# foldl/chatllm.cpp

Measured on AMD Instinct MI355X. Metric: decode tokens/s, higher is better.
Workload: dtype int8xint4 dot / f32 accumulate (Q8_K x Q4_K); 1 GPU; llama3-8b shapes, Q4_K weights, single-token decode, batch 1, 16-token prompt, F16 KV cache; parallelism=single GPU, n_ctx_end=1630

## Files before the change

chatllm.cpp_amd/csrc/decode_fused.hip:

```cpp
#include "common.h"
#include "quant_dev.h"
#include "q4k.h"
#include "dequant.h"

#include <math.h>

__device__ __forceinline__ float lane_xor4_ff(float v) { return __int_as_float(lane_xor4_i(__float_as_int(v))); }
__device__ __forceinline__ float vd32_reduce(float a0, float a1) {
    a0 = a0 + dpp_f<DPP_ROW_ROR8>(a0); a1 = a1 + dpp_f<DPP_ROW_ROR8>(a1);
    a0 = a0 + lane_xor4_ff(a0);        a1 = a1 + lane_xor4_ff(a1);
    a0 = a0 + dpp_f<DPP_QUAD_XOR2>(a0); a1 = a1 + dpp_f<DPP_QUAD_XOR2>(a1);
    const float u = a0 + a1;
    return u + dpp_f<DPP_QUAD_XOR1>(u);
}

static float * g_attn_dbg = nullptr;
static unsigned long long * g_attn_ts = nullptr;
extern "C" __attribute__((visibility("default"))) void cllm_debug_set_attn_ts(unsigned long long * dev_buf) { g_attn_ts = dev_buf; }
extern "C" __attribute__((visibility("default"))) void cllm_debug_set_attn_probs(float * dev_buf) { g_attn_dbg = dev_buf; }

template <bool ROPE>
__global__ void __launch_bounds__(1024) k_attn_decode(const float * __restrict__ qkv, const int32_t * __restrict__ pos_dev, int nh, int nkv, int hd,
                                                      float scale, uint16_t * __restrict__ k_cache, uint16_t * __restrict__ v_cache,
                                                      int64_t ML, float * __restrict__ att, float * __restrict__ dbg, int mode, float theta_scale) {
// ... 118 lines not shown
    const int np = n_kv & ~31, ntail = n_kv - np;
    for (int d0 = wave * 4 + sub; d0 < hd; d0 += nrg) {
        const uint16_t * vr = v_cache + ((int64_t) g * hd + d0) * ML;
        const float vfresh = ROPE ? vnew[d0] : 0.0f;
        float a0 = 0.0f, a1 = 0.0f;
        for (int e = 2 * c16; e < np; e += 32) {
            const float v0 = (ROPE && e == pos) ? vfresh : h2f(vr[e]), v1 = (ROPE && e + 1 == pos) ? vfresh : h2f(vr[e + 1]);
            a0 = __builtin_fmaf(v0, sc[e], a0); a1 = __builtin_fmaf(v1, sc[e + 1], a1);
        }
        const float res = vd32_reduce(a0, a1);
        for (int t = 0; t < 2; t++) {
            const int e = np + 2 * c16 + t;
            if (e < n_kv) tailp[2 * c16 + t] = ((ROPE && e == pos) ? vfresh : h2f(vr[e])) * sc[e];
        }
        wave_lds_fence();
        if (c16 == 0) {
            double s = (double) res;
            for (int t = 0; t < ntail; t++) s += (double) tailp[t];
            att[h * hd + d0] = (float) s;
        }
        wave_lds_fence();
    }
}

__global__ void __launch_bounds__(64) k_rope_table(const int32_t * __restrict__ pos_dev, int half, float theta_scale, float * __restrict__ cs) {
    for (int i = threadIdx.x; i < half; i += 64) {
        float theta = (float) pos_dev[0];
        for (int k = 0; k < i; k++) theta *= theta_scale;
        float c, s_;
        rope_cos_sin(theta, &c, &s_);
        cs[2*i] = c * 1.0f; cs[2*i + 1] = s_ * 1.0f;
    }
}
int launch_rope_table(hipStream_t st, const int32_t * pos_dev, int hd, float freq_base, float * cs) {
    hipLaunchKernelGGL(k_rope_table, dim3(1), dim3(64), 0, st, pos_dev, hd / 2, powf(freq_base, -2.0f / hd), cs);
    LAUNCH_CHECK();
    return CLLM_OK;
}

__device__ __forceinline__ int uniform_load_i32(const int32_t * p) {
    int v;
    asm volatile("s_load_dword %0, %1, 0x0\n\ts_waitcnt lgkmcnt(0)" : "=s"(v) : "s"(p) : "memory");
    return v;
}

template <int HD, int MODE, int PARTS>
__global__ void __launch_bounds__(1024) k_attn_dec(const float * __restrict__ qkv, const int32_t * __restrict__ pos_dev, const float * __restrict__ rope_cs,
                                                   int nh, int nkv, float scale, uint16_t * __restrict__ k_cache, uint16_t * __restrict__ v_cache,
                                                   int ML, float * __restrict__ att, unsigned long long * ts) {
#define TS(k) do { if (ts && threadIdx.x == 0) ts[(blockIdx.y * gridDim.x + blockIdx.x) * 8 + (k)] = wall_clock64(); } while (0)
    extern __shared__ __attribute__((aligned(16))) float sm[];
    __shared__ float  red_f[16];
    __shared__ uint64_t etab_s[32];
    constexpr int half = HD / 2, off = MODE == 0 ? 1 : half, U = 4;
    const int r2 = gridDim.x, g = blockIdx.y, h = g * r2 + blockIdx.x;
    const int tid = threadIdx.x, lane = tid & 63, wave = tid >> 6;
    const int KD = nkv * HD, QD = nh * HD;
    float * qs = sm; float * knew = sm + HD; float * vnew = sm + 2 * HD; float * sc = sm + 3 * HD;

    float px0 = 0.0f, px1 = 0.0f, pc = 0.0f, ps = 0.0f;
    const bool is_pair = tid < 2 * half, is_v = !is_pair && tid < 2 * half + HD;
    const int which = tid >= half ? 1 : 0, pi = tid - which * half, ic = MODE == 0 ? 2 * pi : pi;
    if (is_pair) {
        const float * x = which == 0 ? qkv + h * HD : qkv + QD + g * HD;
        px0 = x[ic]; px1 = x[ic + off];
        pc = rope_cs[2 * pi]; ps = rope_cs[2 * pi + 1];
    } else if (is_v) px0 = qkv[QD + KD + g * HD + (tid - 2 * half)];
    const int pos = uniform_load_i32(pos_dev);
// ... 251 lines not shown
__global__ void __launch_bounds__(256) k_argmax_partial(const float * __restrict__ x, int n, float * __restrict__ pv, int * __restrict__ pi) {
    __shared__ float bv[4]; __shared__ int bi[4];
    const int per = (n + gridDim.x - 1) / gridDim.x;
    const int lo = blockIdx.x * per, hi = min(n, lo + per);
    float best = -INFINITY; int idx = 0x7fffffff;
    for (int i = lo + threadIdx.x; i < hi; i += 256) { const float v = x[i]; if (v > best) { best = v; idx = i; } }
#pragma unroll
    for (int o = 32; o > 0; o >>= 1) argmax_combine(best, idx, __shfl_xor(best, o, 64), __shfl_xor(idx, o, 64));
    if ((threadIdx.x & 63) == 0) { bv[threadIdx.x >> 6] = best; bi[threadIdx.x >> 6] = idx; }
    __syncthreads();
    if (threadIdx.x == 0) {
        for (int w = 1; w < 4; w++) argmax_combine(best, idx, bv[w], bi[w]);
        pv[blockIdx.x] = best; pi[blockIdx.x] = idx;
    }
}
__global__ void __launch_bounds__(256) k_argmax_final(const float * __restrict__ pv, const int * __restrict__ pi, int np, int32_t * __restrict__ tok_dev,
                                                      int32_t * __restrict__ pos_dev, int32_t * __restrict__ out_ring, int32_t * __restrict__ counter) {
    __shared__ float bv[4]; __shared__ int bi[4];
    float best = -INFINITY; int idx = 0x7fffffff;
    for (int i = threadIdx.x; i < np; i += 256) argmax_combine(best, idx, pv[i], pi[i]);
#pragma unroll
    for (int o = 32; o > 0; o >>= 1) argmax_combine(best, idx, __shfl_xor(best, o, 64), __shfl_xor(idx, o, 64));
    if ((threadIdx.x & 63) == 0) { bv[threadIdx.x >> 6] = best; bi[threadIdx.x >> 6] = idx; }
    __syncthreads();
    if (threadIdx.x == 0) {
        for (int w = 1; w < 4; w++) argmax_combine(best, idx, bv[w], bi[w]);
        if (idx == 0x7fffffff) idx = 0;
        tok_dev[0] = idx;
        pos_dev[0] = pos_dev[0] + 1;
        out_ring[counter[0]] = idx;
        counter[0] = counter[0] + 1;
    }
}
__global__ void __launch_bounds__(1024) k_argmax_final_next(const float * __restrict__ pv, const int * __restrict__ pi, int np, int32_t * __restrict__ tok_dev,
                                                            int32_t * __restrict__ pos_dev, int32_t * __restrict__ out_ring, int32_t * __restrict__ counter,
                                                            int etype, const char * __restrict__ emb, size_t emb_nb1, int H, float * __restrict__ x_next,
                                                            int half, float theta_scale, float * __restrict__ cs) {
    __shared__ float bv[16]; __shared__ int bi[16]; __shared__ int tok_s;
    const int tid = threadIdx.x;
    const int pos_next = pos_dev[0] + 1;
    float best = -INFINITY; int idx = 0x7fffffff;
    for (int i = tid; i < np; i += 1024) argmax_combine(best, idx, pv[i], pi[i]);
#pragma unroll
    for (int o = 32; o > 0; o >>= 1) argmax_combine(best, idx, __shfl_xor(best, o, 64), __shfl_xor(idx, o, 64));
    if ((tid & 63) == 0) { bv[tid >> 6] = best; bi[tid >> 6] = idx; }
    __syncthreads();
    if (tid == 0) {
        for (int w = 1; w < 16; w++) argmax_combine(best, idx, bv[w], bi[w]);
        if (idx == 0x7fffffff) idx = 0;
        tok_s = idx;
        tok_dev[0] = idx;
        pos_dev[0] = pos_next;
        out_ring[counter[0]] = idx;
        counter[0] = counter[0] + 1;
    }
    if (cs && tid >= 960)
        for (int i = tid - 960; i < half; i += 64) {
            float theta = (float) pos_next;
            for (int k = 0; k < i; k++) theta *= theta_scale;
            float c, s_;
            rope_cos_sin(theta, &c, &s_);
            cs[2*i] = c * 1.0f; cs[2*i + 1] = s_ * 1.0f;
        }
    __syncthreads();
    const char * row = emb + (size_t) tok_s * emb_nb1;
    for (int c = tid; c < H; c += 1024) x_next[c] = dequant_elem(etype, row, c);
}
int launch_argmax_partial(hipStream_t st, const float * logits, int n, float * part_v, int * part_i) {
    hipLaunchKernelGGL(k_argmax_partial, dim3(256), dim3(256), 0, st, logits, n, part_v, part_i);
    LAUNCH_CHECK();
    return CLLM_OK;
}
int launch_argmax_final_next(hipStream_t st, const float * part_v, const int * part_i, int np, int32_t * tok_dev, int32_t * pos_dev, int32_t * out_ring, int32_t * counter,
                             int etype, const void * emb, size_t emb_nb1, int H, float * x_next, int hd, float freq_base, float * cs) {
    hipLaunchKernelGGL(k_argmax_final_next, dim3(1), dim3(1024), 0, st, part_v, part_i, np, tok_dev, pos_dev, out_ring, counter, etype, (const char *) emb, emb_nb1, H, x_next,
                       hd / 2, hd ? powf(freq_base, -2.0f / hd) : 0.0f, hd ? cs : (float *) nullptr);
    LAUNCH_CHECK();
    return CLLM_OK;
}
__global__ void __launch_bounds__(256) k_argmax_publish(const float * __restrict__ pv, const int * __restrict__ pi, int np, int32_t * __restrict__ tok_dev,
                                                        int32_t * __restrict__ tok_host, int32_t * const * __restrict__ inc, int n_inc) {
    __shared__ float bv[4]; __shared__ int bi[4];
    float best = -INFINITY; int idx = 0x7fffffff;
    for (int i = threadIdx.x; i < np; i += 256) argmax_combine(best, idx, pv[i], pi[i]);
#pragma unroll
    for (int o = 32; o > 0; o >>= 1) argmax_combine(best, idx, __shfl_xor(best, o, 64), __shfl_xor(idx, o, 64));
    if ((threadIdx.x & 63) == 0) { bv[threadIdx.x >> 6] = best; bi[threadIdx.x >> 6] = idx; }
    __syncthreads();
    if (threadIdx.x == 0) {
        for (int w = 1; w < 4; w++) argmax_combine(best, idx, bv[w], bi[w]);
        if (idx == 0x7fffffff) idx = 0;
        tok_dev[0] = idx;
        if (tok_host) { tok_host[0] = idx; __threadfence_system(); }
    }
    for (int i = threadIdx.x; i < n_inc; i += 256) inc[i][0] = inc[i][0] + 1;
}
struct argmax_set_rec { int32_t * ptr; int32_t val; int32_t pad; };
__global__ void __launch_bounds__(256) k_argmax_publish_set(const float * __restrict__ pv, const int * __restrict__ pi, int np, int32_t * __restrict__ tok_dev,
                                                            int32_t * __restrict__ tok_host, const argmax_set_rec * __restrict__ recs, int n_set) {
    __shared__ float bv[4]; __shared__ int bi[4];
    float best = -INFINITY; int idx = 0x7fffffff;
    for (int i = threadIdx.x; i < np; i += 256) argmax_combine(best, idx, pv[i], pi[i]);
#pragma unroll
    for (int o = 32; o > 0; o >>= 1) argmax_combine(best, idx, __shfl_xor(best, o, 64), __shfl_xor(idx, o, 64));
    if ((threadIdx.x & 63) == 0) { bv[threadIdx.x >> 6] = best; bi[threadIdx.x >> 6] = idx; }
    __syncthreads();
    if (threadIdx.x == 0) {
        for (int w = 1; w < 4; w++) argmax_combine(best, idx, bv[w], bi[w]);
        if (idx == 0x7fffffff) idx = 0;
        tok_dev[0] = idx;
        if (tok_host) { tok_host[0] = idx; __threadfence_system(); }
// ... 88 lines not shown
```

chatllm.cpp_amd/lib.py:

```python
import ctypes as C
import os
import subprocess

HERE = os.path.dirname(os.path.abspath(__file__))
SO_PATH = os.environ.get("CLLM_LIB") or os.path.join(HERE, "libchatllm_hip.so")
HEADER = os.path.join(os.path.dirname(HERE), "include", "chatllm_hip.h")


class CllmError(RuntimeError):

    def __init__(self, msg, rc=None):
        super().__init__(msg)
        self.rc = rc


class CTensor(C.Structure):
    _fields_ = [("type", C.c_int32), ("ne", C.c_int64 * 4), ("nb", C.c_size_t * 4), ("data", C.c_void_p)]


class RopeParams(C.Structure):
    _fields_ = [("n_dims", C.c_int32), ("mode", C.c_int32), ("n_ctx_orig", C.c_int32), ("freq_base", C.c_float),
                ("freq_scale", C.c_float), ("ext_factor", C.c_float), ("attn_factor", C.c_float),
                ("beta_fast", C.c_float), ("beta_slow", C.c_float)]

# ... 36 lines not shown
    "cllm_scratch_release": (C.c_int, [_P]),
    "cllm_check_kernel_errors": (C.c_int, []),
    "cllm_graph_capture_begin": (C.c_int, [_P]),
    "cllm_graph_capture_end": (C.c_int, [_P, C.POINTER(C.c_void_p)]),
    "cllm_graph_launch": (C.c_int, [_P, _P]),
    "cllm_graph_destroy": (C.c_int, [_P]),
    "cllm_event_create": (C.c_int, [C.POINTER(C.c_void_p)]),
    "cllm_event_destroy": (C.c_int, [_P]),
    "cllm_event_record": (C.c_int, [_P, _P]),
    "cllm_event_sync": (C.c_int, [_P]),
    "cllm_stream_wait_event": (C.c_int, [_P, _P]),
    "cllm_memcpy_peer_async": (C.c_int, [_P, C.c_int, _P, C.c_int, C.c_size_t, _P]),
    "cllm_event_elapsed_ms": (C.c_int, [_P, _P, C.POINTER(C.c_float)]),
    "cllm_mul_mat_wsize": (C.c_size_t, [_T, _T]),
    "cllm_op_mul_mat": (C.c_int, [_P, _T, _T, _T, _P, C.c_size_t]),
    "cllm_mul_mat_ex_min_cols": (C.c_int, []),
    "cllm_set_prefill_mode": (C.c_int, [C.c_int]),
    "cllm_get_prefill_mode": (C.c_int, []),
    "cllm_set_prefill_attn_mode": (C.c_int, [C.c_int]),
    "cllm_op_mul_mat_ex": (C.c_int, [_P, _T, _T, _T, _P, C.c_size_t, C.c_int, _T, C.c_float, C.c_int, _T]),
    "cllm_set_decode_free_order": (C.c_int, [C.c_int]),
    "cllm_get_decode_free_order": (C.c_int, []),
    "cllm_op_mul_mat_vec_fused": (C.c_int, [_P, _T, C.c_int, _P, _P, C.c_float, C.c_int, _P, _P]),
    "cllm_pack_rows": (C.c_int, [_P, _P, C.POINTER(C.c_void_p), C.POINTER(C.c_int64), C.c_int, C.c_size_t, C.c_int]),
    "cllm_bench_mul_mat_kernel": (C.c_int, [_P, _T, C.POINTER(C.c_void_p), C.c_int, _T, _T, _P, C.c_size_t, C.c_int, C.POINTER(C.c_float)]),
    "cllm_bench_mul_mat_id": (C.c_int, [_P, _T, _T, _T, C.POINTER(C.c_void_p), C.c_int, _T, _P, C.c_size_t, C.c_int, C.POINTER(C.c_float)]),
    "cllm_bench_read_bw": (C.c_int, [_P, C.c_size_t, C.c_int, C.POINTER(C.c_float)]),
    "cllm_bench_gemv_fused": (C.c_int, [_P, C.c_int, C.POINTER(C.c_void_p), C.c_int, C.c_int64, C.c_int64, C.c_int, _P, _P, C.c_float, C.c_int, _P, _P, C.c_int,
                                        C.POINTER(C.c_float)]),
    "cllm_op_mul_mat_id": (C.c_int, [_P, _T, _T, _T, _T, _P, C.c_size_t]),
    "cllm_op_argmax_advance": (C.c_int, [_P, _P, C.c_int64, _P, _P, _P, C.c_int, _P]),
    "cllm_op_argmax_set": (C.c_int, [_P, _P, C.c_int64, _P, _P, _P, C.c_int, _P]),
    "cllm_op_snapshot_argmax_set": (C.c_int, [_P, _P, C.c_int, _P, C.c_int64, _P, _P, _P, C.c_int, _P]),
    "cllm_flash_attn_wsize": (C.c_size_t, [_T]),
    "cllm_op_flash_attn_ext": (C.c_int, [_P, _T, _T, _T, _T, _T, C.c_float, C.c_float, C.c_float, _P, C.c_size_t]),
    "cllm_attn_prefill_min_cols": (C.c_int, []),
    "cllm_op_attn_prefill": (C.c_int, [_P, _T, _T, _T, _T, C.c_float, C.c_int]),
    "cllm_op_mul_mat_id_silu_mul": (C.c_int, [_P, _T, _T, _T, _T]),
    "cllm_quantize_row_q8_0": (C.c_int, [_P, _P, _P, C.c_int64]),
    "cllm_quantize_row_q8_1": (C.c_int, [_P, _P, _P, C.c_int64]),
    "cllm_quantize_row_q8_K": (C.c_int, [_P, _P, _P, C.c_int64]),
    "cllm_vec_dot_isums": (C.c_int, [_P, C.c_int, C.c_int64, _P, _P, _P]),
    "cllm_op_rms_norm": (C.c_int, [_P, _T, _T, C.c_float]),
    "cllm_op_rms_norm_mul": (C.c_int, [_P, _T, _T, _T, C.c_float]),
    "cllm_op_rope": (C.c_int, [_P, _T, _T, _T, _T, C.POINTER(RopeParams)]),
    "cllm_op_soft_max": (C.c_int, [_P, _T, _T, _T, C.c_float, C.c_float]),
    "cllm_op_diag_mask_inf": (C.c_int, [_P, _T, _T, C.c_int]),
    "cllm_op_scale": (C.c_int, [_P, _T, _T, C.c_float, C.c_float]),
    "cllm_op_scale_mask_soft_max": (C.c_int, [_P, _T, _T, C.c_float, C.c_int]),
    "cllm_op_attn_decode": (C.c_int, [_P, _P, _P, C.c_int, C.c_int, C.c_int, _P, _P, C.c_int64, _P]),
    "cllm_op_rope_table": (C.c_int, [_P, _P, C.c_int, C.c_float, _P]),
    "cllm_attn_decode_supported": (C.c_int, [C.c_int, C.c_int, C.c_int, C.c_int64]),
    "cllm_attn_decode_wsize": (C.c_size_t, [C.c_int64, C.c_int, C.c_int64]),
    "cllm_op_rope_kv_attn_decode": (C.c_int, [_P, _P, _P, _P, C.c_float, C.c_int64, C.c_int, C.c_int, C.c_int, C.c_int, _P, _P, C.c_int64, _P, _P, C.c_size_t]),
    "cllm_op_unary": (C.c_int, [_P, C.c_int, _T, _T]),
    "cllm_op_sqr": (C.c_int, [_P, _T, _T]),
    "cllm_op_add": (C.c_int, [_P, _T, _T, _T]),
    "cllm_op_mul": (C.c_int, [_P, _T, _T, _T]),
    "cllm_op_div": (C.c_int, [_P, _T, _T, _T]),
    "cllm_op_sum_rows": (C.c_int, [_P, _T, _T]),
    "cllm_op_top_k": (C.c_int, [_P, _T, _T]),
    "cllm_op_moe_combine": (C.c_int, [_P, _T, _T, _T, _T, _T]),
    "cllm_op_mul_mat_id_combine": (C.c_int, [_P, _T, _T, _T, _T, _T, _T]),
    "cllm_op_moe_router": (C.c_int, [_P, _T, _T, C.c_float, _T, _T, _T, _T]),
    "cllm_op_moe_router_gate_up": (C.c_int, [_P, _T, _T, C.c_float, _T, _T, _T, _T, _T]),
    "cllm_op_silu_mul": (C.c_int, [_P, _T, _T, _T]),
# ... 92 lines not shown
```

include/chatllm_hip.h:

```cpp
#ifndef CHATLLM_HIP_H
#define CHATLLM_HIP_H

#include <stddef.h>
#include <stdint.h>

#ifdef __cplusplus
extern "C" {
#endif

#define CLLM_API __attribute__((visibility("default")))

typedef enum cllm_status {
    CLLM_OK            =  0,
    CLLM_E_INVALID     = -1,
    CLLM_E_UNSUPPORTED = -2,
    CLLM_E_HIP         = -3,
    CLLM_E_ALLOC       = -4,
} cllm_status;

typedef enum cllm_type {
    CLLM_TYPE_F32 = 0, CLLM_TYPE_F16 = 1, CLLM_TYPE_Q4_0 = 2, CLLM_TYPE_Q4_1 = 3, CLLM_TYPE_Q8_0 = 8, CLLM_TYPE_Q4_K = 12, CLLM_TYPE_Q5_K = 13, CLLM_TYPE_Q6_K = 14,
    CLLM_TYPE_Q5_0 = 6, CLLM_TYPE_Q5_1 = 7, CLLM_TYPE_Q2_K = 10, CLLM_TYPE_Q3_K = 11, CLLM_TYPE_IQ4_NL = 20, CLLM_TYPE_IQ2_XXS = 16, CLLM_TYPE_IQ2_XS = 17, CLLM_TYPE_IQ3_XXS = 18, CLLM_TYPE_IQ1_S = 19, CLLM_TYPE_IQ3_S = 21, CLLM_TYPE_IQ2_S = 22, CLLM_TYPE_IQ4_XS = 23, CLLM_TYPE_IQ1_M = 29, CLLM_TYPE_TQ1_0 = 34, CLLM_TYPE_TQ2_0 = 35, CLLM_TYPE_MXFP4 = 39,
    CLLM_TYPE_I32 = 26, CLLM_TYPE_I64 = 27,
} cllm_type;
// ... 80 lines not shown

CLLM_API int    cllm_quantize_row_q8_0(void * stream, const float * x, void * y_blocks, int64_t k);
CLLM_API int    cllm_quantize_row_q8_1(void * stream, const float * x, void * y_blocks, int64_t k);
CLLM_API int    cllm_quantize_row_q8_K(void * stream, const float * x, void * y_blocks, int64_t k);
CLLM_API int    cllm_vec_dot_isums(void * stream, int wtype, int64_t k, const void * w_row, const float * x, int32_t * isums);

CLLM_API int cllm_op_rms_norm(void * stream, const cllm_tensor * src, cllm_tensor * dst, float eps);
CLLM_API int cllm_op_rms_norm_mul(void * stream, const cllm_tensor * src, const cllm_tensor * weight, cllm_tensor * dst, float eps);

typedef struct cllm_rope_params {
    int32_t n_dims, mode, n_ctx_orig;
    float   freq_base, freq_scale, ext_factor, attn_factor, beta_fast, beta_slow;
} cllm_rope_params;
CLLM_API int cllm_op_rope(void * stream, const cllm_tensor * src, const cllm_tensor * pos, const cllm_tensor * freq_factors,
                          cllm_tensor * dst, const cllm_rope_params * p);
CLLM_API int cllm_op_soft_max(void * stream, const cllm_tensor * src, const cllm_tensor * mask, cllm_tensor * dst,
                              float scale, float max_bias);
CLLM_API int cllm_op_diag_mask_inf(void * stream, const cllm_tensor * src, cllm_tensor * dst, int n_past);
CLLM_API int cllm_op_scale(void * stream, const cllm_tensor * src, cllm_tensor * dst, float s, float b);
CLLM_API int cllm_op_scale_mask_soft_max(void * stream, const cllm_tensor * src, cllm_tensor * dst, float scale, int n_past);

CLLM_API size_t cllm_flash_attn_wsize(const cllm_tensor * q);
CLLM_API int    cllm_op_flash_attn_ext(void * stream, const cllm_tensor * q, const cllm_tensor * k, const cllm_tensor * v, const cllm_tensor * mask,
                                       cllm_tensor * dst, float scale, float max_bias, float logit_softcap, void * wdata, size_t wsize);
CLLM_API int    cllm_attn_prefill_min_cols(void);
CLLM_API int    cllm_op_attn_prefill(void * stream, const cllm_tensor * q, const cllm_tensor * k, const cllm_tensor * vt, cllm_tensor * dst,
                                     float scale, int n_past);

CLLM_API int cllm_op_argmax_advance(void * stream, const float * logits, int64_t n, int32_t * tok_dev, int32_t * tok_host,
                                    int32_t * const * inc_ptrs_dev, int n_inc, void * scratch);
CLLM_API int cllm_op_argmax_set(void * stream, const float * logits, int64_t n, int32_t * tok_dev, int32_t * tok_host, const void * set_table_dev, int n_set, void * scratch);
CLLM_API int cllm_op_snapshot_argmax_set(void * stream, const void * ranges_dev, int n_ranges, const float * logits, int64_t n, int32_t * tok_dev, int32_t * tok_host,
                                         const void * set_table_dev, int n_set, void * scratch);

CLLM_API int cllm_op_attn_decode(void * stream, const float * q, const int32_t * pos_dev, int n_head, int n_kv_head, int head_dim,
                                 const void * k_cache, const void * v_cache, int64_t max_len, float * out);

CLLM_API int    cllm_op_rope_table(void * stream, const int32_t * pos_dev, int head_dim, float freq_base, float * cs );
CLLM_API int    cllm_attn_decode_supported(int n_head, int n_kv_head, int head_dim, int64_t max_len);
CLLM_API size_t cllm_attn_decode_wsize(int64_t n_kv, int n_head, int64_t max_len);
CLLM_API int    cllm_op_rope_kv_attn_decode(void * stream, const float * qkv, const int32_t * pos_dev, const float * rope_cs, float freq_base, int64_t n_kv,
                                            int n_head, int n_kv_head, int head_dim, int rope_mode, void * k_cache, void * v_cache, int64_t max_len,
                                            float * out, void * wdata, size_t wsize);

typedef enum cllm_unary {
    CLLM_UNARY_TANH = 4, CLLM_UNARY_RELU = 6, CLLM_UNARY_SIGMOID = 7, CLLM_UNARY_GELU = 8, CLLM_UNARY_GELU_QUICK = 9, CLLM_UNARY_SILU = 10,
} cllm_unary;
CLLM_API int cllm_op_unary(void * stream, int op, const cllm_tensor * src, cllm_tensor * dst);
CLLM_API int cllm_op_sqr(void * stream, const cllm_tensor * src, cllm_tensor * dst);
CLLM_API int cllm_op_add(void * stream, const cllm_tensor * a, const cllm_tensor * b, cllm_tensor * dst);
CLLM_API int cllm_op_mul(void * stream, const cllm_tensor * a, const cllm_tensor * b, cllm_tensor * dst);
CLLM_API int cllm_op_div(void * stream, const cllm_tensor * a, const cllm_tensor * b, cllm_tensor * dst);
CLLM_API int cllm_op_sum_rows(void * stream, const cllm_tensor * src, cllm_tensor * dst);
CLLM_API int cllm_op_top_k(void * stream, const cllm_tensor * src, cllm_tensor * dst);
CLLM_API int cllm_op_moe_combine(void * stream, const cllm_tensor * experts, const cllm_tensor * probs, const cllm_tensor * ids, const cllm_tensor * resid,
                                 cllm_tensor * dst);
CLLM_API int cllm_op_mul_mat_id_combine(void * stream, const cllm_tensor * as, const cllm_tensor * b, const cllm_tensor * ids, const cllm_tensor * probs,
                                        const cllm_tensor * resid, cllm_tensor * dst);
CLLM_API int cllm_op_moe_router_gate_up(void * stream, const cllm_tensor * x, const cllm_tensor * norm_w, float eps, const cllm_tensor * gate_w, const cllm_tensor * as_gu,
                                        cllm_tensor * probs, cllm_tensor * ids, cllm_tensor * dst);
CLLM_API int cllm_op_moe_router(void * stream, const cllm_tensor * x, const cllm_tensor * norm_w, float eps, const cllm_tensor * gate_w,
                                cllm_tensor * xnorm, cllm_tensor * probs, cllm_tensor * ids);
CLLM_API int cllm_op_silu_mul(void * stream, const cllm_tensor * gate, const cllm_tensor * up, cllm_tensor * dst);

CLLM_API int cllm_op_set_rows(void * stream, const cllm_tensor * src, const cllm_tensor * idx, cllm_tensor * dst);
CLLM_API int cllm_op_cpy(void * stream, const cllm_tensor * src, cllm_tensor * dst);
// ... 68 lines not shown
```

Baseline: 667.3 tokens/s.

## Specialize argmax-final-next kernel per embedding type with warp-split roles and LDS row staging

Adds a templated 320-thread version of the final argmax kernel. Four wavefronts reduce the argmax in a single shuffle pass and stage the chosen embedding row in LDS, while a fifth wavefront advances the position and computes the rope table concurrently. Q4_K rows are dequantized eight values per thread with vectorized stores, which replaces the per-element dequant over 1024 threads and one of the barriers. The change also adds timestamp probes, a flag to force the generic path, and public C entry points; the kernel is one small launch per token, so its effect on overall decode speed is limited.

```diff
diff --git a/chatllm.cpp_amd/csrc/decode_fused.hip b/chatllm.cpp_amd/csrc/decode_fused.hip
--- a/chatllm.cpp_amd/csrc/decode_fused.hip
+++ b/chatllm.cpp_amd/csrc/decode_fused.hip
@@ -493,19 +493,29 @@
         counter[0] = counter[0] + 1;
     }
 }
+static unsigned long long * g_final_ts = nullptr;
+static bool g_final_generic = false;
+extern "C" __attribute__((visibility("default"))) void cllm_debug_set_final_ts(unsigned long long * dev_buf) { g_final_ts = dev_buf; }
+extern "C" __attribute__((visibility("default"))) void cllm_debug_set_final_generic(int on) { g_final_generic = on != 0; }
+#define FTS(k) do { if (ts) ts[(k)] = wall_clock64(); } while (0)
 __global__ void __launch_bounds__(1024) k_argmax_final_next(const float * __restrict__ pv, const int * __restrict__ pi, int np, int32_t * __restrict__ tok_dev,
                                                             int32_t * __restrict__ pos_dev, int32_t * __restrict__ out_ring, int32_t * __restrict__ counter,
                                                             int etype, const char * __restrict__ emb, size_t emb_nb1, int H, float * __restrict__ x_next,
-                                                            int half, float theta_scale, float * __restrict__ cs) {
+                                                            int half, float theta_scale, float * __restrict__ cs, unsigned long long * __restrict__ ts) {
     __shared__ float bv[16]; __shared__ int bi[16]; __shared__ int tok_s;
     const int tid = threadIdx.x;
+    unsigned long long * const ts_all = ts;
+    if (tid) ts = nullptr;
+    FTS(0);
     const int pos_next = pos_dev[0] + 1;
     float best = -INFINITY; int idx = 0x7fffffff;
     for (int i = tid; i < np; i += 1024) argmax_combine(best, idx, pv[i], pi[i]);
 #pragma unroll
     for (int o = 32; o > 0; o >>= 1) argmax_combine(best, idx, __shfl_xor(best, o, 64), __shfl_xor(idx, o, 64));
     if ((tid & 63) == 0) { bv[tid >> 6] = best; bi[tid >> 6] = idx; }
-    __syncthreads();
+    FTS(1);
+    __syncthreads();
+    FTS(2);
     if (tid == 0) {
         for (int w = 1; w < 16; w++) argmax_combine(best, idx, bv[w], bi[w]);
         if (idx == 0x7fffffff) idx = 0;
@@ -515,7 +525,8 @@
         out_ring[counter[0]] = idx;
         counter[0] = counter[0] + 1;
     }
-    if (cs && tid >= 960)
+    FTS(3);
+    if (cs && tid >= 960) {
         for (int i = tid - 960; i < half; i += 64) {
             float theta = (float) pos_next;
             for (int k = 0; k < i; k++) theta *= theta_scale;
@@ -523,19 +534,136 @@
             rope_cos_sin(theta, &c, &s_);
             cs[2*i] = c * 1.0f; cs[2*i + 1] = s_ * 1.0f;
         }
-    __syncthreads();
+        if (ts_all && tid == 960) ts_all[6] = wall_clock64();
+    }
+    __syncthreads();
+    FTS(4);
     const char * row = emb + (size_t) tok_s * emb_nb1;
     for (int c = tid; c < H; c += 1024) x_next[c] = dequant_elem(etype, row, c);
+    FTS(5);
 }
 int launch_argmax_partial(hipStream_t st, const float * logits, int n, float * part_v, int * part_i) {
     hipLaunchKernelGGL(k_argmax_partial, dim3(256), dim3(256), 0, st, logits, n, part_v, part_i);
     LAUNCH_CHECK();
     return CLLM_OK;
 }
+static __device__ __noinline__ float2 rope_cos_sin_v(float theta) {
+    float2 r;
+    r.x = gm_cosf(theta);
+    r.y = gm_sinf(theta);
+    return r;
+}
+__device__ __forceinline__ void q4k_row_decode8(const char * row, int g, float * __restrict__ x) {
+    const uint32_t * blk = (const uint32_t *)(row + (size_t)(g >> 5) * 144);
+    const int r = g & 31, j = r >> 3, l = (r & 7) * 4;
+    const uint32_t dm = blk[0], s0 = blk[1], s1 = blk[2], s2 = blk[3], q = blk[4 + 8 * j + (r & 7)];
+    auto sb = [&](int i) { const uint32_t w = i < 4 ? s0 : i < 8 ? s1 : s2; return (int)((w >> (8 * (i & 3))) & 0xff); };
+    float d1[2], m1[2];
+#pragma unroll
+    for (int h = 0; h < 2; h++) {
+        const int s = 2 * j + h;
+        int sc, m;
+        if (s < 4) { sc = sb(s) & 63; m = sb(s + 4) & 63; }
+        else { sc = (sb(s + 4) & 0xF) | ((sb(s - 4) >> 6) << 4); m = (sb(s + 4) >> 4) | ((sb(s) >> 6) << 4); }
+        d1[h] = h2f((uint16_t)(dm & 0xffff)) * (float) sc; m1[h] = h2f((uint16_t)(dm >> 16)) * (float) m;
+    }
+    float4 lo, hi;
+    lo.x = d1[0] * (float)((q      ) & 0xF) - m1[0]; hi.x = d1[1] * (float)((q >>  4) & 0xF) - m1[1];
+    lo.y = d1[0] * (float)((q >>  8) & 0xF) - m1[0]; hi.y = d1[1] * (float)((q >> 12) & 0xF) - m1[1];
+    lo.z = d1[0] * (float)((q >> 16) & 0xF) - m1[0]; hi.z = d1[1] * (float)((q >> 20) & 0xF) - m1[1];
+    lo.w = d1[0] * (float)((q >> 24) & 0xF) - m1[0]; hi.w = d1[1] * (float)((q >> 28) & 0xF) - m1[1];
+    float * o = x + (size_t)(g >> 5) * 256 + 64 * j + l;
+    *(float4 *) o = lo; *(float4 *)(o + 32) = hi;
+}
+template <int ETYPE>
+__global__ void __launch_bounds__(320) k_argmax_final_next_t(const float * __restrict__ pv, const int * __restrict__ pi, int np, int32_t * __restrict__ tok_dev,
+                                                             int32_t * __restrict__ pos_dev, int32_t * __restrict__ out_ring, int32_t * __restrict__ counter,
+                                                             const char * __restrict__ emb, size_t emb_nb1, int H, float * __restrict__ x_next,
+                                                             int half, float theta_scale, float * __restrict__ cs, unsigned long long * __restrict__ ts) {
+    extern __shared__ u32x4 row_s[];
+    const int tid = threadIdx.x, lane = tid & 63;
+    unsigned long long * const ts_all = ts;
+    if (tid) ts = nullptr;
+    FTS(0);
+    if (tid >= 256) {
+        const int pos_next = uniform_load_i32(pos_dev) + 1;
+        if (lane == 0) pos_dev[0] = pos_next;
+        if (cs) {
+            for (int i = lane; i < half; i += 64) {
+                float theta = (float) pos_next;
+                for (int k = 0; k < i; k++) theta *= theta_scale;
+                const float2 r = rope_cos_sin_v(theta);
+                cs[2*i] = r.x * 1.0f; cs[2*i + 1] = r.y * 1.0f;
+            }
+            if (ts_all && lane == 0) ts_all[6] = wall_clock64();
+        }
+    } else {
+        float v[4]; int id[4];
+#pragma unroll
+        for (int k = 0; k < 4; k++) { const int i = lane + 64 * k; const bool in = i < np; v[k] = in ? pv[i] : -INFINITY; id[k] = in ? pi[i] : 0x7fffffff; }
+        float best = -INFINITY; int idx = 0x7fffffff;
+#pragma unroll
+        for (int k = 0; k < 4; k++) argmax_combine(best, idx, v[k], id[k]);
+#pragma unroll
+        for (int o = 32; o > 0; o >>= 1) argmax_combine(best, idx, __shfl_xor(best, o, 64), __shfl_xor(idx, o, 64));
+        const int tok = __builtin_amdgcn_readfirstlane(idx == 0x7fffffff ? 0 : idx);
+        FTS(1);
+        const u32x4 * row = (const u32x4 *)(emb + (size_t) tok * emb_nb1);
+        const int n16 = (int)(emb_nb1 >> 4);
+        for (int i = tid; i < n16; i += 256) row_s[i] = row[i];
+        if (tid == 0) {
+            tok_dev[0] = tok;
+            out_ring[counter[0]] = tok;
+            counter[0] = counter[0] + 1;
+            FTS(3);
+        }
+    }
+    __syncthreads();
+    FTS(4);
+    if (tid < 256) {
+        if constexpr (ETYPE == CLLM_TYPE_Q4_K) {
+            for (int g = tid; g < (H >> 3); g += 256) q4k_row_decode8((const char *) row_s, g, x_next);
+        } else {
+            for (int c4 = tid; c4 < (H >> 2); c4 += 256) {
+                float4 o;
+                o.x = dequant_elem(ETYPE, (const char *) row_s, 4 * c4);     o.y = dequant_elem(ETYPE, (const char *) row_s, 4 * c4 + 1);
+                o.z = dequant_elem(ETYPE, (const char *) row_s, 4 * c4 + 2); o.w = dequant_elem(ETYPE, (const char *) row_s, 4 * c4 + 3);
+                ((float4 *) x_next)[c4] = o;
+            }
+        }
+    }
+    FTS(5);
+}
 int launch_argmax_final_next(hipStream_t st, const float * part_v, const int * part_i, int np, int32_t * tok_dev, int32_t * pos_dev, int32_t * out_ring, int32_t * counter,
                              int etype, const void * emb, size_t emb_nb1, int H, float * x_next, int hd, float freq_base, float * cs) {
+    const int half = hd / 2; const float theta_scale = hd ? powf(freq_base, -2.0f / hd) : 0.0f;
+    float * const csp = hd ? cs : (float *) nullptr;
+    const bool fits = !g_final_generic && np <= 256 && H % 4 == 0 && emb_nb1 % 16 == 0 && emb_nb1 <= 65536 && emb_nb1 == cllm_row_size(etype, H) &&
+                      ((uintptr_t) emb | (uintptr_t) x_next) % 16 == 0;
+#define FINAL_T(T_) case T_: hipLaunchKernelGGL(k_argmax_final_next_t<T_>, dim3(1), dim3(320), emb_nb1, st, part_v, part_i, np, tok_dev, pos_dev, out_ring, counter, (const char *) emb, \
+                                                emb_nb1, H, x_next, half, theta_scale, csp, g_final_ts); LAUNCH_CHECK(); return CLLM_OK
+    if (fits) switch (etype) {
+        FINAL_T(CLLM_TYPE_F32); FINAL_T(CLLM_TYPE_F16); FINAL_T(CLLM_TYPE_Q8_0); FINAL_T(CLLM_TYPE_Q4_0); FINAL_T(CLLM_TYPE_Q4_1); FINAL_T(CLLM_TYPE_Q4_K); FINAL_T(CLLM_TYPE_Q6_K);
+        default: break;
+    }
+#undef FINAL_T
     hipLaunchKernelGGL(k_argmax_final_next, dim3(1), dim3(1024), 0, st, part_v, part_i, np, tok_dev, pos_dev, out_ring, counter, etype, (const char *) emb, emb_nb1, H, x_next,
-                       hd / 2, hd ? powf(freq_base, -2.0f / hd) : 0.0f, hd ? cs : (float *) nullptr);
+                       half, theta_scale, csp, g_final_ts);
+    LAUNCH_CHECK();
+    return CLLM_OK;
+}
+extern "C" int cllm_op_argmax_final_next(void * stream, const float * part_v, const int * part_i, int np, int32_t * tok_dev, int32_t * pos_dev, int32_t * out_ring, int32_t * counter,
+                                         int etype, const void * emb, int64_t H, float * x_next, int head_dim, float freq_base, float * cs) {
+    if (!part_v || !part_i || np < 0 || !tok_dev || !pos_dev || !out_ring || !counter || !emb || H <= 0 || H > INT32_MAX || !x_next || head_dim < 0 || head_dim % 2 ||
+        (head_dim && !cs))
+        FAIL(CLLM_E_INVALID, "argmax_final_next: arguments");
+    const int bs = cllm_blck_size(etype);
+    if (bs <= 0 || H % bs) FAIL(CLLM_E_INVALID, "argmax_final_next: %lld elements are not whole blocks of type %d", (long long) H, etype);
+    return launch_argmax_final_next((hipStream_t) stream, part_v, part_i, np, tok_dev, pos_dev, out_ring, counter, etype, emb, cllm_row_size(etype, H), (int) H, x_next, head_dim, freq_base, cs);
+}
+extern "C" int cllm_op_argmax_final(void * stream, const float * part_v, const int * part_i, int np, int32_t * tok_dev, int32_t * pos_dev, int32_t * out_ring, int32_t * counter) {
+    if (!part_v || !part_i || np < 0 || !tok_dev || !pos_dev || !out_ring || !counter) FAIL(CLLM_E_INVALID, "argmax_final: arguments");
+    hipLaunchKernelGGL(k_argmax_final, dim3(1), dim3(256), 0, (hipStream_t) stream, part_v, part_i, np, tok_dev, pos_dev, out_ring, counter);
     LAUNCH_CHECK();
     return CLLM_OK;
 }
diff --git a/chatllm.cpp_amd/lib.py b/chatllm.cpp_amd/lib.py
--- a/chatllm.cpp_amd/lib.py
+++ b/chatllm.cpp_amd/lib.py
@@ -92,6 +92,8 @@
     "cllm_op_argmax_advance": (C.c_int, [_P, _P, C.c_int64, _P, _P, _P, C.c_int, _P]),
     "cllm_op_argmax_set": (C.c_int, [_P, _P, C.c_int64, _P, _P, _P, C.c_int, _P]),
     "cllm_op_snapshot_argmax_set": (C.c_int, [_P, _P, C.c_int, _P, C.c_int64, _P, _P, _P, C.c_int, _P]),
+    "cllm_op_argmax_final": (C.c_int, [_P, _P, _P, C.c_int, _P, _P, _P, _P]),
+    "cllm_op_argmax_final_next": (C.c_int, [_P, _P, _P, C.c_int, _P, _P, _P, _P, C.c_int, _P, C.c_int64, _P, C.c_int, C.c_float, _P]),
     "cllm_flash_attn_wsize": (C.c_size_t, [_T]),
     "cllm_op_flash_attn_ext": (C.c_int, [_P, _T, _T, _T, _T, _T, C.c_float, C.c_float, C.c_float, _P, C.c_size_t]),
     "cllm_attn_prefill_min_cols": (C.c_int, []),
diff --git a/include/chatllm_hip.h b/include/chatllm_hip.h
--- a/include/chatllm_hip.h
+++ b/include/chatllm_hip.h
@@ -136,6 +136,9 @@
 CLLM_API int cllm_op_argmax_set(void * stream, const float * logits, int64_t n, int32_t * tok_dev, int32_t * tok_host, const void * set_table_dev, int n_set, void * scratch);
 CLLM_API int cllm_op_snapshot_argmax_set(void * stream, const void * ranges_dev, int n_ranges, const float * logits, int64_t n, int32_t * tok_dev, int32_t * tok_host,
                                          const void * set_table_dev, int n_set, void * scratch);
+CLLM_API int cllm_op_argmax_final(void * stream, const float * part_v, const int * part_i, int np, int32_t * tok_dev, int32_t * pos_dev, int32_t * out_ring, int32_t * counter);
+CLLM_API int cllm_op_argmax_final_next(void * stream, const float * part_v, const int * part_i, int np, int32_t * tok_dev, int32_t * pos_dev, int32_t * out_ring, int32_t * counter,
+                                       int etype, const void * emb, int64_t H, float * x_next, int head_dim, float freq_base, float * cs);
 
 CLLM_API int cllm_op_attn_decode(void * stream, const float * q, const int32_t * pos_dev, int n_head, int n_kv_head, int head_dim,
                                  const void * k_cache, const void * v_cache, int64_t max_len, float * out);
```

After: 669.5 tokens/s (median of 6 runs). About the same (+0.3%).

## Restructure argmax tail kernel into barrier-free wave-specialized roles with typed embedding dequant

Applied to the files above, without the earlier changes.

Rewrites the final argmax + next-token embedding kernel so it no longer uses __syncthreads. Each wave recomputes the argmax redundantly over the partials with DPP reductions, then dequantizes the embedding row with vectorized type-specialized paths (Q4_K etc.). Separate waves handle the pos/rope-table update and the token/ring bookkeeping. Host powf is cached, and new C entry points are exported. The aim is to cut serial latency in a small single-block kernel on the decode critical path, at the cost of redundant argmax reads and more code paths.

```diff
diff --git a/chatllm.cpp_amd/csrc/decode_fused.hip b/chatllm.cpp_amd/csrc/decode_fused.hip
--- a/chatllm.cpp_amd/csrc/decode_fused.hip
+++ b/chatllm.cpp_amd/csrc/decode_fused.hip
@@ -174,8 +174,14 @@
         cs[2*i] = c * 1.0f; cs[2*i + 1] = s_ * 1.0f;
     }
 }
+static float rope_theta_scale(float freq_base, int hd) {
+    static thread_local float base = 0.0f, scale = 0.0f;
+    static thread_local int size = 0;
+    if (base != freq_base || size != hd) { scale = powf(freq_base, -2.0f / hd); base = freq_base; size = hd; }
+    return scale;
+}
 int launch_rope_table(hipStream_t st, const int32_t * pos_dev, int hd, float freq_base, float * cs) {
-    hipLaunchKernelGGL(k_rope_table, dim3(1), dim3(64), 0, st, pos_dev, hd / 2, powf(freq_base, -2.0f / hd), cs);
+    hipLaunchKernelGGL(k_rope_table, dim3(1), dim3(64), 0, st, pos_dev, hd / 2, rope_theta_scale(freq_base, hd), cs);
     LAUNCH_CHECK();
     return CLLM_OK;
 }
@@ -493,39 +499,116 @@
         counter[0] = counter[0] + 1;
     }
 }
-__global__ void __launch_bounds__(1024) k_argmax_final_next(const float * __restrict__ pv, const int * __restrict__ pi, int np, int32_t * __restrict__ tok_dev,
-                                                            int32_t * __restrict__ pos_dev, int32_t * __restrict__ out_ring, int32_t * __restrict__ counter,
-                                                            int etype, const char * __restrict__ emb, size_t emb_nb1, int H, float * __restrict__ x_next,
+#define TAIL_ROW_THREADS 512
+template <int ETYPE> __device__ __forceinline__ void tail_row(int etype, const char * __restrict__ row, int H, float * __restrict__ x, int t) {
+    if (ETYPE == CLLM_TYPE_Q4_K) {
+        for (int u = t; u < (H >> 8) * 32; u += TAIL_ROW_THREADS) {
+            const int b = u >> 5, j = (u >> 3) & 3, k = u & 7;
+            const char * blk = row + (size_t) b * 144;
+            const u32x4 h = *(const u32x4 *) blk;
+            const uint32_t q = *(const uint32_t *)(blk + 16 + 32 * j + 4 * k);
+            const unsigned long long s8 = h.y | ((unsigned long long) h.z << 32);
+            auto sbyte = [&](int i) { return (int)((i < 8 ? (uint32_t)(s8 >> (8 * i)) : h.w >> (8 * (i - 8))) & 0xff); };
+            const float d = h2f((uint16_t)(h.x & 0xffff)), dmin = h2f((uint16_t)(h.x >> 16));
+            f32x4 o[2];
+#pragma unroll
+            for (int p = 0; p < 2; p++) {
+                const int s = 2 * j + p;
+                int sc, m;
+                if (s < 4) { sc = sbyte(s) & 63; m = sbyte(s + 4) & 63; }
+                else { sc = (sbyte(s + 4) & 0xF) | ((sbyte(s - 4) >> 6) << 4); m = (sbyte(s + 4) >> 4) | ((sbyte(s) >> 6) << 4); }
+                const float d1 = d * (float) sc, m1 = dmin * (float) m;
+#pragma unroll
+                for (int e = 0; e < 4; e++) o[p][e] = d1 * (float)((q >> (8 * e + 4 * p)) & 0xF) - m1;
+            }
+            *(f32x4 *)(x + 256 * b + 64 * j + 4 * k) = o[0];
+            *(f32x4 *)(x + 256 * b + 64 * j + 32 + 4 * k) = o[1];
+        }
+    } else if (ETYPE == CLLM_TYPE_Q4_0) {
+        for (int u = t; u < (H >> 5) * 4; u += TAIL_ROW_THREADS) {
+            const int b = u >> 2, k = u & 3;
+            const uint16_t * blk = (const uint16_t *)(row + (size_t) b * 18);
+            const float d = h2f(blk[0]);
+            const uint32_t q = blk[1 + 2 * k] | ((uint32_t) blk[2 + 2 * k] << 16);
+            f32x4 lo, hi;
+#pragma unroll
+            for (int e = 0; e < 4; e++) { lo[e] = (float)((int)((q >> (8 * e)) & 0xF) - 8) * d; hi[e] = (float)((int)((q >> (8 * e + 4)) & 0xF) - 8) * d; }
+            *(f32x4 *)(x + 32 * b + 4 * k) = lo;
+            *(f32x4 *)(x + 32 * b + 16 + 4 * k) = hi;
+        }
+    } else if (ETYPE == CLLM_TYPE_Q8_0) {
+        for (int u = t; u < (H >> 5) * 8; u += TAIL_ROW_THREADS) {
+            const int b = u >> 3, k = u & 7;
+            const uint16_t * blk = (const uint16_t *)(row + (size_t) b * 34);
+            const float d = h2f(blk[0]);
+            const uint32_t q = blk[1 + 2 * k] | ((uint32_t) blk[2 + 2 * k] << 16);
+            f32x4 o;
+#pragma unroll
+            for (int e = 0; e < 4; e++) o[e] = (float)(int8_t)((q >> (8 * e)) & 0xff) * d;
+            *(f32x4 *)(x + 32 * b + 4 * k) = o;
+        }
+    } else if (ETYPE == CLLM_TYPE_F16) {
+        for (int u = t; u < (H >> 2); u += TAIL_ROW_THREADS) {
+            const u32x2 w = ((const u32x2 *) row)[u];
+            f32x4 o;
+            o[0] = h2f((uint16_t)(w.x & 0xffff)); o[1] = h2f((uint16_t)(w.x >> 16)); o[2] = h2f((uint16_t)(w.y & 0xffff)); o[3] = h2f((uint16_t)(w.y >> 16));
+            ((f32x4 *) x)[u] = o;
+        }
+    } else if (ETYPE == CLLM_TYPE_F32) {
+        for (int u = t; u < (H >> 2); u += TAIL_ROW_THREADS) ((f32x4 *) x)[u] = ((const f32x4 *) row)[u];
+    } else {
+        for (int c = t; c < H; c += TAIL_ROW_THREADS) x[c] = dequant_elem(etype, row, c);
+    }
+}
+__device__ __forceinline__ void argmax_take(float & best, int & idx, float ov, int oi) {
+    const bool t = (ov > best) | ((ov == best) & (oi < idx));
+    best = t ? ov : best; idx = t ? oi : idx;
+}
+__device__ __forceinline__ int tail_argmax(const float * __restrict__ pv, const int * __restrict__ pi, int np, int lane) {
+    float v[4]; int ix[4];
+#pragma unroll
+    for (int r = 0; r < 4; r++) { const int i = lane + 64 * r, ic = i < np ? i : 0; v[r] = pv[ic]; ix[r] = pi[ic]; }
+    float best = -INFINITY; int idx = 0x7fffffff;
+#pragma unroll
+    for (int r = 0; r < 4; r++) if (lane + 64 * r < np) argmax_take(best, idx, v[r], ix[r]);
+    for (int i = lane + 256; i < np; i += 64) argmax_take(best, idx, pv[i], pi[i]);
+    argmax_take(best, idx, dpp_f<DPP_QUAD_XOR1>(best), dpp_i<DPP_QUAD_XOR1>(idx));
+    argmax_take(best, idx, dpp_f<DPP_QUAD_XOR2>(best), dpp_i<DPP_QUAD_XOR2>(idx));
+    argmax_take(best, idx, dpp_f<DPP_HALF_MIRROR>(best), dpp_i<DPP_HALF_MIRROR>(idx));
+    argmax_take(best, idx, dpp_f<DPP_ROW_MIRROR>(best), dpp_i<DPP_ROW_MIRROR>(idx));
+    float wb = lane_f(best, 0); int tok = __builtin_amdgcn_readlane(idx, 0);
+#pragma unroll
+    for (int r = 1; r < 4; r++) argmax_take(wb, tok, lane_f(best, 16 * r), __builtin_amdgcn_readlane(idx, 16 * r));
+    return tok == 0x7fffffff ? 0 : tok;
+}
+template <int ETYPE>
+__global__ void __launch_bounds__(TAIL_ROW_THREADS + 128) k_argmax_final_next(const float * __restrict__ pv, const int * __restrict__ pi, const char * __restrict__ emb, size_t emb_nb1,
+                                                            float * __restrict__ x_next, int np, int H, int32_t * __restrict__ counter, int32_t * __restrict__ pos_dev,
+                                                            int32_t * __restrict__ tok_dev, int32_t * __restrict__ out_ring, int etype,
                                                             int half, float theta_scale, float * __restrict__ cs) {
-    __shared__ float bv[16]; __shared__ int bi[16]; __shared__ int tok_s;
-    const int tid = threadIdx.x;
-    const int pos_next = pos_dev[0] + 1;
-    float best = -INFINITY; int idx = 0x7fffffff;
-    for (int i = tid; i < np; i += 1024) argmax_combine(best, idx, pv[i], pi[i]);
-#pragma unroll
-    for (int o = 32; o > 0; o >>= 1) argmax_combine(best, idx, __shfl_xor(best, o, 64), __shfl_xor(idx, o, 64));
-    if ((tid & 63) == 0) { bv[tid >> 6] = best; bi[tid >> 6] = idx; }
-    __syncthreads();
-    if (tid == 0) {
-        for (int w = 1; w < 16; w++) argmax_combine(best, idx, bv[w], bi[w]);
-        if (idx == 0x7fffffff) idx = 0;
-        tok_s = idx;
-        tok_dev[0] = idx;
-        pos_dev[0] = pos_next;
-        out_ring[counter[0]] = idx;
-        counter[0] = counter[0] + 1;
-    }
-    if (cs && tid >= 960)
-        for (int i = tid - 960; i < half; i += 64) {
-            float theta = (float) pos_next;
-            for (int k = 0; k < i; k++) theta *= theta_scale;
-            float c, s_;
-            rope_cos_sin(theta, &c, &s_);
-            cs[2*i] = c * 1.0f; cs[2*i + 1] = s_ * 1.0f;
-        }
-    __syncthreads();
-    const char * row = emb + (size_t) tok_s * emb_nb1;
-    for (int c = tid; c < H; c += 1024) x_next[c] = dequant_elem(etype, row, c);
+    const int tid = threadIdx.x, lane = tid & 63;
+    if (tid < TAIL_ROW_THREADS) {
+        const int tok = tail_argmax(pv, pi, np, lane);
+        tail_row<ETYPE>(etype, emb + (size_t) tok * emb_nb1, H, x_next, tid);
+    } else if (tid < TAIL_ROW_THREADS + 64) {
+        const int pos_next = pos_dev[0] + 1;
+        if (lane == 0) pos_dev[0] = pos_next;
+        if (cs)
+            for (int i = lane; i < half; i += 64) {
+                float theta = (float) pos_next;
+                for (int k = 0; k < i; k++) theta *= theta_scale;
+                const float c = gm_cosf(theta), s_ = gm_sinf(theta);
+                cs[2*i] = c * 1.0f; cs[2*i + 1] = s_ * 1.0f;
+            }
+    } else {
+        const int cnt = __hip_atomic_load(counter, __ATOMIC_RELAXED, __HIP_MEMORY_SCOPE_AGENT);
+        const int tok = tail_argmax(pv, pi, np, lane);
+        if (lane == 0) {
+            tok_dev[0] = tok;
+            out_ring[cnt] = tok;
+            counter[0] = cnt + 1;
+        }
+    }
 }
 int launch_argmax_partial(hipStream_t st, const float * logits, int n, float * part_v, int * part_i) {
     hipLaunchKernelGGL(k_argmax_partial, dim3(256), dim3(256), 0, st, logits, n, part_v, part_i);
@@ -534,10 +617,47 @@
 }
 int launch_argmax_final_next(hipStream_t st, const float * part_v, const int * part_i, int np, int32_t * tok_dev, int32_t * pos_dev, int32_t * out_ring, int32_t * counter,
                              int etype, const void * emb, size_t emb_nb1, int H, float * x_next, int hd, float freq_base, float * cs) {
-    hipLaunchKernelGGL(k_argmax_final_next, dim3(1), dim3(1024), 0, st, part_v, part_i, np, tok_dev, pos_dev, out_ring, counter, etype, (const char *) emb, emb_nb1, H, x_next,
-                       hd / 2, hd ? powf(freq_base, -2.0f / hd) : 0.0f, hd ? cs : (float *) nullptr);
-    LAUNCH_CHECK();
-    return CLLM_OK;
+    const uintptr_t al = (uintptr_t) emb | (uintptr_t) emb_nb1;
+    int body = -1;
+    if (((uintptr_t) x_next & 15) == 0) {
+        if      (etype == CLLM_TYPE_Q4_K && H % 256 == 0 && (al & 15) == 0) body = CLLM_TYPE_Q4_K;
+        else if (etype == CLLM_TYPE_Q4_0 && H % 32 == 0 && (al & 1) == 0)   body = CLLM_TYPE_Q4_0;
+        else if (etype == CLLM_TYPE_Q8_0 && H % 32 == 0 && (al & 1) == 0)   body = CLLM_TYPE_Q8_0;
+        else if (etype == CLLM_TYPE_F16 && H % 4 == 0 && (al & 7) == 0)     body = CLLM_TYPE_F16;
+        else if (etype == CLLM_TYPE_F32 && H % 4 == 0 && (al & 15) == 0)    body = CLLM_TYPE_F32;
+    }
+    const float theta_scale = hd ? rope_theta_scale(freq_base, hd) : 0.0f;
+#define GO(ETYPE_) hipLaunchKernelGGL(k_argmax_final_next<ETYPE_>, dim3(1), dim3(TAIL_ROW_THREADS + 128), 0, st, part_v, part_i, (const char *) emb, emb_nb1, x_next, np, H, counter, pos_dev, \
+                                      tok_dev, out_ring, etype, hd / 2, theta_scale, hd ? cs : (float *) nullptr)
+    switch (body) {
+        case CLLM_TYPE_Q4_K: GO(CLLM_TYPE_Q4_K); break;
+        case CLLM_TYPE_Q4_0: GO(CLLM_TYPE_Q4_0); break;
+        case CLLM_TYPE_Q8_0: GO(CLLM_TYPE_Q8_0); break;
+        case CLLM_TYPE_F16:  GO(CLLM_TYPE_F16);  break;
+        case CLLM_TYPE_F32:  GO(CLLM_TYPE_F32);  break;
+        default:             GO(-1);             break;
+    }
+#undef GO
+    LAUNCH_CHECK();
+    return CLLM_OK;
+}
+extern "C" int cllm_op_argmax_partial(void * stream, const float * logits, int64_t n, float * part_v, int32_t * part_i) {
+    if (!logits || n <= 0 || n > INT32_MAX || !part_v || !part_i) FAIL(CLLM_E_INVALID, "argmax_partial: arguments");
+    return launch_argmax_partial((hipStream_t) stream, logits, (int) n, part_v, (int *) part_i);
+}
+extern "C" int cllm_op_argmax_final(void * stream, const float * part_v, const int32_t * part_i, int np, int32_t * tok_dev, int32_t * pos_dev, int32_t * out_ring, int32_t * counter) {
+    if (!part_v || !part_i || np <= 0 || !tok_dev || !pos_dev || !out_ring || !counter) FAIL(CLLM_E_INVALID, "argmax_final: arguments");
+    hipLaunchKernelGGL(k_argmax_final, dim3(1), dim3(256), 0, (hipStream_t) stream, part_v, (const int *) part_i, np, tok_dev, pos_dev, out_ring, counter);
+    LAUNCH_CHECK();
+    return CLLM_OK;
+}
+extern "C" int cllm_op_argmax_final_next(void * stream, const float * part_v, const int32_t * part_i, int np, int32_t * tok_dev, int32_t * pos_dev, int32_t * out_ring, int32_t * counter,
+                                         const cllm_tensor * emb, float * x_next, int head_dim, float freq_base, float * cs) {
+    if (!part_v || !part_i || np <= 0 || !tok_dev || !pos_dev || !out_ring || !counter || !emb || !emb->data || !x_next || emb->ne[0] <= 0 || emb->ne[0] > INT32_MAX)
+        FAIL(CLLM_E_INVALID, "argmax_final_next: arguments");
+    if (head_dim < 0 || head_dim % 2 || (head_dim && !cs)) FAIL(CLLM_E_INVALID, "argmax_final_next: head_dim %d", head_dim);
+    return launch_argmax_final_next((hipStream_t) stream, part_v, (const int *) part_i, np, tok_dev, pos_dev, out_ring, counter, emb->type, emb->data, emb->nb[1], (int) emb->ne[0],
+                                    x_next, head_dim, freq_base, cs);
 }
 __global__ void __launch_bounds__(256) k_argmax_publish(const float * __restrict__ pv, const int * __restrict__ pi, int np, int32_t * __restrict__ tok_dev,
                                                         int32_t * __restrict__ tok_host, int32_t * const * __restrict__ inc, int n_inc) {
diff --git a/chatllm.cpp_amd/lib.py b/chatllm.cpp_amd/lib.py
--- a/chatllm.cpp_amd/lib.py
+++ b/chatllm.cpp_amd/lib.py
@@ -92,6 +92,9 @@
     "cllm_op_argmax_advance": (C.c_int, [_P, _P, C.c_int64, _P, _P, _P, C.c_int, _P]),
     "cllm_op_argmax_set": (C.c_int, [_P, _P, C.c_int64, _P, _P, _P, C.c_int, _P]),
     "cllm_op_snapshot_argmax_set": (C.c_int, [_P, _P, C.c_int, _P, C.c_int64, _P, _P, _P, C.c_int, _P]),
+    "cllm_op_argmax_partial": (C.c_int, [_P, _P, C.c_int64, _P, _P]),
+    "cllm_op_argmax_final": (C.c_int, [_P, _P, _P, C.c_int, _P, _P, _P, _P]),
+    "cllm_op_argmax_final_next": (C.c_int, [_P, _P, _P, C.c_int, _P, _P, _P, _P, _T, _P, C.c_int, C.c_float, _P]),
     "cllm_flash_attn_wsize": (C.c_size_t, [_T]),
     "cllm_op_flash_attn_ext": (C.c_int, [_P, _T, _T, _T, _T, _T, C.c_float, C.c_float, C.c_float, _P, C.c_size_t]),
     "cllm_attn_prefill_min_cols": (C.c_int, []),
diff --git a/include/chatllm_hip.h b/include/chatllm_hip.h
--- a/include/chatllm_hip.h
+++ b/include/chatllm_hip.h
@@ -136,6 +136,11 @@
 CLLM_API int cllm_op_argmax_set(void * stream, const float * logits, int64_t n, int32_t * tok_dev, int32_t * tok_host, const void * set_table_dev, int n_set, void * scratch);
 CLLM_API int cllm_op_snapshot_argmax_set(void * stream, const void * ranges_dev, int n_ranges, const float * logits, int64_t n, int32_t * tok_dev, int32_t * tok_host,
                                          const void * set_table_dev, int n_set, void * scratch);
+CLLM_API int cllm_op_argmax_partial(void * stream, const float * logits, int64_t n, float * part_v , int32_t * part_i );
+CLLM_API int cllm_op_argmax_final(void * stream, const float * part_v, const int32_t * part_i, int np, int32_t * tok_dev, int32_t * pos_dev, int32_t * out_ring,
+                                  int32_t * counter);
+CLLM_API int cllm_op_argmax_final_next(void * stream, const float * part_v, const int32_t * part_i, int np, int32_t * tok_dev, int32_t * pos_dev, int32_t * out_ring,
+                                       int32_t * counter, const cllm_tensor * emb, float * x_next, int head_dim, float freq_base, float * cs );
 
 CLLM_API int cllm_op_attn_decode(void * stream, const float * q, const int32_t * pos_dev, int n_head, int n_kv_head, int head_dim,
                                  const void * k_cache, const void * v_cache, int64_t max_len, float * out);
```

Result: no change. 671.6 tokens/s before, 674.5 tokens/s after, median of 3 (+0.4%).
